# Manta-Network/manta-rs

Hardware: AMD Instinct MI355X
Metric: G1 MSM Mscalar/s at 2^20 (higher is better)
Workload: dtype u32; 1 GPU; 2^20 BLS12-381 G1 variable-base MSM per GPU, uniform scalars resident in HBM; curve=BLS12-381, log_n=20, window_bits=17, msms_in_flight=3

## Files before the change

include/mantagpu.h:

```cpp
#ifndef MANTAGPU_H
#define MANTAGPU_H
#include <stddef.h>
#include <stdint.h>

#ifdef __cplusplus
extern "C" {
#endif

typedef enum { MG_BN254 = 0, MG_BLS12_381 = 1 } mg_curve_t;

enum {
    MG_SUCCESS = 0,
    MG_ERROR_INVALID_ARGUMENT = 1,
    MG_ERROR_HIP = 2,
    MG_ERROR_OUT_OF_MEMORY = 3,
    MG_ERROR_DOMAIN_TOO_LARGE = 4,
    MG_ERROR_STATE = 5,
    MG_ERROR_CHECKSUM = 6
};

typedef struct mg_bases mg_bases;
typedef struct mg_msm_job mg_msm_job;
typedef struct mg_ctx mg_ctx;

// ... 22 lines not shown
int mg_bases_create_sharded(mg_curve_t curve, int group, const uint64_t *affine_mont, size_t n, const int *devices,
                            int n_devices, int precompute_window_bits, mg_bases **out);
int mg_bases_num_shards(const mg_bases *bases);
int mg_bases_shard(const mg_bases *bases, int shard, int *device, size_t *lo, size_t *hi);
void mg_bases_destroy(mg_bases *bases);
size_t mg_bases_device_bytes(const mg_bases *bases);
int mg_msm(const mg_bases *bases, const uint64_t *scalars_canonical, size_t n, uint64_t *out_affine_mont);
#define MG_SCALARS_MONT 1
#define MG_SCALARS_SPARSE 2
int mg_msm_launch(const mg_bases *bases, const uint64_t *d_scalars, size_t n, int scalar_flags, int window_bits,
                  mg_msm_job **job);
int mg_msm_launch_sharded(const mg_bases *bases, const uint64_t *const *d_scalars_per_shard, int scalar_flags,
                          int window_bits, mg_msm_job **job);
int mg_msm_finish(mg_msm_job *job, uint64_t *out_affine_mont);
int mg_msm_result_to_device(mg_msm_job *job, uint64_t *d_out_xyzz, void *stream);
size_t mg_xyzz_limbs(mg_curve_t curve, int group);
int mg_xyzz_sum(mg_curve_t curve, int group, const uint64_t *xyzz, size_t n, uint64_t *out_affine_mont);
int mg_points_sum(mg_curve_t curve, int group, const uint64_t *affine_mont, size_t n, uint64_t *out_affine_mont);
int mg_fixed_base_mul(mg_curve_t curve, int group, const uint64_t *base_affine_mont, const uint64_t *d_scalars,
                      size_t n, uint64_t *d_out_affine_mont);
#define MG_EC_ADD_MIXED 0
#define MG_EC_ADD 1
#define MG_EC_DOUBLE 2
#define MG_EC_MUL 3
#define MG_EC_SUB_MIXED 4
#define MG_EC_MUL_FIXED 5
int mg_ec_elementwise(mg_curve_t curve, int group, int op, const uint64_t *a_affine, const uint64_t *b, size_t n,
                      uint64_t *out_affine);
#define MG_FIELD_ADD 0
#define MG_FIELD_SUB 1
// ... 187 lines not shown
```

manta_rs_amd/api.py:

```python
from __future__ import annotations

import ctypes
import os

import numpy as np

_HERE = os.path.dirname(os.path.abspath(__file__))
LIB_PATH = os.environ.get("MANTA_LIB") or os.path.join(_HERE, "lib", "libmantagpu.so")

BN254, BLS12_381 = 0, 1
FQ_LIMBS = {BN254: 4, BLS12_381: 6}


class MantaGpuError(RuntimeError):

    def __init__(self, status, where=""):
        self.status = status
        detail = LIB.mg_last_error().decode() if status == 2 else ""
        super().__init__(f"{where}: {LIB.mg_strerror(status).decode()} ({status}) {detail}")


def _load():
    if not os.path.exists(LIB_PATH):
        raise ImportError(
# ... 30 lines not shown
    "mg_ntt_device", "mg_groth16_setup", "mg_ctx_create", "mg_ctx_create_from_bytes", "mg_ctx_set_r1cs", "mg_groth16_prove", "mg_groth16_prove_batch", "mg_witness_map", "mg_ctx_domain_size", "mg_ctx_table_bytes",
    "mg_ctx_destroy", "mg_bases_create_sharded", "mg_bases_num_shards", "mg_bases_shard", "mg_msm_launch_sharded",
    "mg_ctx_create_sharded", "mg_ctx_create_from_bytes_sharded", "mg_ctx_num_variables", "mg_ctx_num_inputs",
    "mg_ctx_num_shards", "mg_field_op", "mg_vk_create", "mg_vk_create_from_bytes", "mg_vk_encoded_size", "mg_vk_encode",
    "mg_vk_alpha_beta", "mg_vk_num_inputs", "mg_vk_destroy", "mg_groth16_verify", "mg_groth16_verify_batch", "mg_pairing_check", "mg_proof_decode", "mg_group_ntt",
    "mg_msm_result_to_device", "mg_xyzz_limbs", "mg_xyzz_sum", "mg_ctx_create_shard", "mg_partials_slot_limbs",
    "mg_groth16_partials_launch", "mg_groth16_partials_finish", "mg_groth16_assemble", "mg_blake3", "mg_ctx_create_from_bytes_checked",
    "mg_last_ntt_ms", "mg_hw_queues", "mg_last_prove_phases_ms", "mg_clock_probe", "mg_last_accumulate_mhz", "mg_ctx_create_task",
    "mg_ctx_opts_init", "mg_ctx_create_ex", "mg_ctx_create_from_bytes_ex", "mg_last_pass_host_ms",
    "mg_tuning_init", "mg_get_tuning", "mg_set_tuning", "mg_tuning_env_names",
    "mg_points_decode", "mg_points_check", "mg_points_encode", "mg_proofs_decode",
    "mg_poseidon_create", "mg_poseidon_destroy", "mg_poseidon_permute", "mg_poseidon_hash", "mg_poseidon_hash_device",
    "mg_merkle_tree", "mg_merkle_forest_roots",
    "mg_edwards_decode", "mg_edwards_encode", "mg_edwards_check", "mg_edwards_mul", "mg_edwards_add",
    "mg_note_cipher_create", "mg_note_cipher_destroy", "mg_notes_encrypt", "mg_notes_decrypt",
]


def _chk(rc, where):
    if rc != 0:
        raise MantaGpuError(rc, where)


def _p(a):
    return None if a is None else a.ctypes.data_as(_vp)


def _u64(a):
    return np.ascontiguousarray(a, dtype=np.uint64)

# ... 185 lines not shown


class MsmJob:
    def __init__(self, bases, handle):
        self.bases, self.handle = bases, handle

    def finish(self):
        out = np.zeros(affine_limbs(self.bases.curve, self.bases.group), dtype=np.uint64)
        _chk(LIB.mg_msm_finish(self.handle, _p(out)), "mg_msm_finish")
        self.handle = None
        return out

    def result_to_device(self, d_out_ptr, stream=None):
        _chk(LIB.mg_msm_result_to_device(self.handle, _addr(d_out_ptr), _addr(stream)), "mg_msm_result_to_device")

    def release(self):
        _chk(LIB.mg_msm_finish(self.handle, None), "mg_msm_finish")
        self.handle = None


class VariableBaseMSM:

    @staticmethod
    def multi_scalar_mul(bases: Bases, scalars) -> np.ndarray:
        sc = _u64(scalars)
        out = np.zeros(affine_limbs(bases.curve, bases.group), dtype=np.uint64)
        _chk(LIB.mg_msm(bases.handle, _p(sc), _sz(sc.shape[0]), _p(out)), "mg_msm")
        return out

    @staticmethod
# ... 1 lines not shown
        ptr = d_scalars.ptr if isinstance(d_scalars, DeviceBuffer) else d_scalars
        h = _vp()
        _chk(LIB.mg_msm_launch(bases.handle, ptr, _sz(n), int(bool(scalars_mont)) | (2 if sparse else 0), int(window_bits),
                               ctypes.byref(h)),
             "mg_msm_launch")
        return MsmJob(bases, h)

    @staticmethod
    def launch_sharded(bases: Bases, d_scalars_per_shard, scalars_mont=False, window_bits=0, sparse=False) -> MsmJob:
        ptrs = [d.ptr if isinstance(d, DeviceBuffer) else d for d in d_scalars_per_shard]
        arr = (_vp * len(ptrs))(*ptrs)
        h = _vp()
        _chk(LIB.mg_msm_launch_sharded(bases.handle, arr, int(bool(scalars_mont)) | (2 if sparse else 0), int(window_bits),
                                       ctypes.byref(h)), "mg_msm_launch_sharded")
        return MsmJob(bases, h)


def blake3(data: bytes) -> bytes:
    out = ctypes.create_string_buffer(32)
    _chk(LIB.mg_blake3(bytes(data), _sz(len(data)), out), "mg_blake3")
    return out.raw


def xyzz_limbs(curve, group) -> int:
    return int(LIB.mg_xyzz_limbs(curve, group))


def xyzz_sum(curve, group, xyzz) -> np.ndarray:
    pts = _u64(xyzz).reshape(-1, xyzz_limbs(curve, group))
    out = np.zeros(affine_limbs(curve, group), dtype=np.uint64)
# ... 707 lines not shown
```

manta_rs_amd/csrc/capi.cpp:

```cpp
#include "../../include/mantagpu.h"
#include "engine.h"
#include "staging.h"
#include "tuning.h"
#include <cstddef>
#include "prover.h"
#include "verify.h"
#include <cstring>
#include <new>
#include <vector>

using namespace mg;

struct BasesShard {
    GroupEngine *eng;
    BaseSet *bs;
    int device;
    size_t lo, hi;
};
struct mg_bases {
    std::vector<BasesShard> sh;
    size_t n = 0;
};
struct JobShard {
    GroupEngine *eng;
// ... 285 lines not shown
}
MG_API int mg_msm_result_to_device(mg_msm_job *job, uint64_t *d_out_xyzz, void *stream) {
    MG_TRY
    if (!job || job->sh.size() != 1 || !d_out_xyzz) return MG_ERROR_INVALID_ARGUMENT;
    JobShard &j = job->sh[0];
    DeviceGuard guard;
    MG_HIP(hipSetDevice(j.device));
    int rc = j.eng->msm_fold_device(j.ws, (u32 *)d_out_xyzz, (size_t)j.eng->xyzz_words());
    if (rc) return rc;
    hipStream_t ms = msm_stream_of(j.ws);
    MG_HIP(hipEventRecord(j.ws->done, ms));
    if ((hipStream_t)stream != ms) MG_HIP(hipStreamWaitEvent((hipStream_t)stream, j.ws->done, 0));
    return MG_SUCCESS;
    MG_CATCH
}
MG_API size_t mg_xyzz_limbs(mg_curve_t curve, int group) {
    GroupEngine *e = get_engine((int)curve, group);
    return e ? (size_t)e->xyzz_words() / 2 : 0;
}
MG_API int mg_xyzz_sum(mg_curve_t curve, int group, const uint64_t *xyzz, size_t n, uint64_t *out_affine) {
    MG_TRY
    GroupEngine *e = get_engine((int)curve, group);
    if (!e || !xyzz || !out_affine) return MG_ERROR_INVALID_ARGUMENT;
    HostPoint acc, t;
    e->hp_set_inf(&acc);
    for (size_t i = 0; i < n; ++i) {
        e->hp_from_xyzz(&t, (const u32 *)xyzz + i * (size_t)e->xyzz_words());
        e->hp_add(&acc, &t);
    }
    e->hp_to_affine(&acc, (u32 *)out_affine);
// ... 587 lines not shown
```

manta_rs_amd/csrc/engine.h:

```cpp
#pragma once
#include <hip/hip_runtime.h>
#include <shared_mutex>
#include <atomic>
#include <cstddef>
#include <cstdint>
#include <mutex>
#include <vector>

namespace mg {

typedef uint32_t u32;
typedef uint64_t u64;

#ifdef MG_NO_PRIO
#define MG_PRIO_HIGH() ((void)0)
#else
#define MG_PRIO_HIGH() __builtin_amdgcn_s_setprio(3)
#endif
#define MG_PRIO_FOR(F) MG_PRIO_HIGH()

enum { MG_OK = 0, MG_ERR_ARG = 1, MG_ERR_HIP = 2, MG_ERR_OOM = 3, MG_ERR_DOMAIN = 4, MG_ERR_STATE = 5 };

void set_last_hip_error(hipError_t e, const char *expr, const char *file, int line);
inline int hip_status(hipError_t e, const char *what, const char *file = __builtin_FILE(), int line = __builtin_LINE()) {
// ... 145 lines not shown
    bool use_solo = false;
    hipStream_t side_stream = nullptr;
    hipEvent_t side_fork = nullptr, side_join = nullptr;
    hipEvent_t done = nullptr;
    hipEvent_t t0 = nullptr, t1 = nullptr;
    bool timed = false;
    bool in_graph_slot = false;
    bool capturing = false;
    bool notify = false;
    u32 *h_flag = nullptr;
    u32 *d_token = nullptr;
    float accumulate_ms = 0.f;
    MsmPlan plan;
    MsmTail tail;
    u32 batch = 1;
    int pending = 0;
    int device = 0;
    ~MsmWorkspace();
};

inline hipStream_t msm_stream_of(const MsmWorkspace *ws) {
    return ws->run_on ? ws->run_on : (ws->use_solo && ws->solo ? ws->solo : ws->stream);
}

struct HostPoint {
    u64 w[4 * 12];
};

class GroupEngine {
  public:
// ... 48 lines not shown
    void ws_release(MsmWorkspace *);

    static constexpr size_t MAX_IDLE_WS = 24;

  protected:
    std::mutex ws_mu_;
    std::vector<MsmWorkspace *> ws_free_;
};

GroupEngine *make_engine_bn254_g1();
GroupEngine *make_engine_bn254_g2();
GroupEngine *make_engine_bls381_g1();
GroupEngine *make_engine_bls381_g2();
GroupEngine *get_engine(int curve, int group);

size_t sort_pairs_temp_bytes(size_t n);
bool sort_pairs_takes_device_count(int end_bit);
int sort_pairs(const u32 *keys_in, u32 *keys_out, const u32 *vals_in, u32 *vals_out, size_t n, int end_bit,
               void *tmp, size_t tmp_bytes, hipStream_t s, const u32 *d_count = nullptr, u32 lowmask = 0xffffffffu,
               u32 inv_from = 0xffffffffu);

}
```

manta_rs_amd/csrc/msm_digits.h:

```cpp
#pragma once
#include "msm_common.h"

namespace mg {

template <class FrC>
__global__ __launch_bounds__(1024) void digits_kernel(const u32 *__restrict__ scalars, u32 n, int c, int W, u32 B,
                                                     int precomp, u32 tstride, int mont, u32 invalid,
                                                     u32 *__restrict__ keys, u32 *__restrict__ vals,
                                                     const u32 *__restrict__ map, u32 n_scalars,
                                                     size_t scalar_stride, u32 seg_keys, u32 *__restrict__ count,
                                                     u32 n_sets = 1, u32 set_len = 0, u32 i_first = 0) {
    MG_PRIO_HIGH();
    const u32 i = i_first + blockIdx.x * blockDim.x + threadIdx.x;
    scalars += (size_t)blockIdx.y * scalar_stride;
    u32 src = (i < n) ? (map ? map[i] : i) : 0xffffffffu;
    u32 set = 0;
    if (n_sets > 1 && i < n) {
        set = src / set_len;
        src -= set * set_len;
    }
    const u32 key0 = (blockIdx.y * n_sets + set) * seg_keys;
    const bool have = i < n && src < n_scalars;
    u32 s[8] = {0, 0, 0, 0, 0, 0, 0, 0};
    if (have && mont == 2) {
        typedef FpR<FrC> R;
        const Fp<FrC> f = R::load(scalars + (size_t)src * R::K).to_canonical();
#pragma unroll
// ... 63 lines not shown
            const size_t o = (size_t)w * n + i;
            keys[o] = d ? key0 + (precomp == 2 ? 0u : precomp ? (d - 1) : ((u32)w * B + d - 1)) : invalid;
            vals[o] = d ? ((precomp == 2 ? ((u32)w * tstride + i) * B + (d - 1) : precomp ? ((u32)w * tstride + i) : i) | ((neg ^ flip) << 31)) : 0;
        }
        return;
    }
    const int lane = threadIdx.x & 63;
    u32 total = 0;
    {
        u32 t[8], carry = 0, neg;
#pragma unroll
        for (int j = 0; j < 8; ++j) t[j] = s[j];
        for (int w = 0; w < W; ++w) total += (u32)__popcll(__ballot(next_digit(t, carry, neg) != 0));
    }
    __shared__ u32 wave_tot[16], block_base;
    const int wv = threadIdx.x >> 6, nwv = blockDim.x >> 6;
    if (lane == 0) wave_tot[wv] = total;
    __syncthreads();
    if (threadIdx.x == 0) {
        u32 t = 0;
        for (int q = 0; q < nwv; ++q) t += wave_tot[q];
        block_base = t ? atomicAdd(count, t) : 0;
    }
    __syncthreads();
    u32 base = block_base;
    for (int q = 0; q < wv; ++q) base += wave_tot[q];
    const unsigned long long lt = (1ull << lane) - 1ull;
    u32 carry = 0, neg;
    for (int w = 0; w < W; ++w) {
        const u32 d = next_digit(s, carry, neg);
        const unsigned long long m = __ballot(d != 0);
        if (d) {
            const u32 o = base + (u32)__popcll(m & lt);
            keys[o] = key0 + (precomp == 2 ? 0u : precomp ? (d - 1) : ((u32)w * B + d - 1));
            vals[o] = (precomp == 2 ? ((u32)w * tstride + i) * B + (d - 1) : precomp ? ((u32)w * tstride + i) : i) | ((neg ^ flip) << 31);
        }
        base += (u32)__popcll(m);
    }
}

}
```

manta_rs_amd/csrc/msm_engine.h:

```cpp
#pragma once
#include "msm_common.h"
#include "staging.h"
#include "msm_digits.h"
#include "msm_accumulate.h"
#include "msm_reduce.h"
#include "msm_tables.h"

namespace mg {

template <class Curve, int GROUP> struct GT;
template <class Curve> struct GT<Curve, 1> {
#ifdef MG_G1_SATURATED
    typedef Fp<typename Curve::Fq> F;
#else
    typedef FpR<typename Curve::Fq> F;
#endif
    typedef Fp<typename Curve::Fq> FIO;
    typedef host::HFp<typename Curve::Fq> HF;
};
template <class Curve> struct GT<Curve, 2> {
#ifdef MG_G2_SATURATED
    typedef Fp2<typename Curve::Fq> F;
#else
    typedef Fp2R<typename Curve::Fq> F;
// ... 4 lines not shown

static inline u32 cdiv(size_t a, size_t b) { return (u32)((a + b - 1) / b); }

static __global__ __launch_bounds__(256) void stage_and_notify_kernel(const u32 *__restrict__ src0, u32 *__restrict__ dst0, u32 n0,
                                                                      const u32 *__restrict__ src1, u32 *__restrict__ dst1, u32 n1,
                                                                      u32 *__restrict__ flag) {
    for (u32 i = threadIdx.x; i < n0; i += 256) dst0[i] = src0[i];
    for (u32 i = threadIdx.x; i < n1; i += 256) dst1[i] = src1[i];
    __threadfence_system();
    __syncthreads();
    if (threadIdx.x == 0 && flag) {
        __atomic_store_n(flag, 1u, __ATOMIC_RELEASE);
        __threadfence_system();
    }
}
struct ZeroRanges {
    u32 *p[3];
    u32 n[3];
};
template <class F> __global__ __launch_bounds__(256) void zero_ranges(ZeroRanges r) {
    const u32 stride = gridDim.x * 256u, i0 = blockIdx.x * 256u + threadIdx.x;
#pragma unroll
    for (int t = 0; t < 3; ++t)
        for (u32 i = i0; i < r.n[t]; i += stride) r.p[t][i] = 0u;
}

static int ab_knob_in(const char *name, int lo, int hi, int dflt) {
    const int v = ab_knob(name, dflt);
    return v < lo ? lo : (v > hi ? hi : v);
}
struct MsmKnobs {
    int msm_L = ab_knob("MANTA_MSM_L", 0);
    int acc_round_waves = ab_knob("MANTA_ACC_ROUND_WAVES", -1);
    int coop_tiles = ab_knob("MANTA_COOP_TILES", 64);
    u32 coop_waves = (u32)ab_knob("MANTA_COOP_WAVES", 512);
    u32 merge_g = [](int v) { return (u32)(v >= 1 && v <= 64 ? v : 0); }(ab_knob("MANTA_MERGE_G", 0));
    int lgS0 = ab_knob_in("MANTA_RED_S0", 1, 8, 2), lgS = ab_knob_in("MANTA_RED_S", -1, 8, -1), lgSP = ab_knob_in("MANTA_RED_SP", 1, 8, 3);
    u32 min_items = (u32)ab_knob_in("MANTA_RED_MIN", 128, 1 << 30, 16384);
    u32 min_items_batch = (u32)ab_knob_in("MANTA_RED_MIN_BATCH", 128, 1 << 30, ab_knob("MANTA_RED_MIN", -1) >= 0 ? (int)min_items : 2048);
    bool side = ab_knob_in("MANTA_RED_SIDE", 0, 1, 1) != 0;
    bool sort_low = ab_knob("MANTA_SORT_LOW", 1) != 0;
    int acc_single = ab_knob("MANTA_ACC_SINGLE", 1);
    u32 digits_threads = [](int v) { return (u32)(v == 256 || v == 512 || v == 1024 ? v : 256); }(ab_knob("MANTA_DIGITS_THREADS", 0));
    bool z3_sort = ab_knob("MANTA_Z3_SORT", 0) != 0;
    size_t fixed_base_table_min = (size_t)ab_knob("MANTA_FIXED_BASE_TABLE_MIN", 16384);
};
static const MsmKnobs &msm_knobs() {
    static const MsmKnobs k;
    return k;
}

template <class Curve, int CURVE_ID, int GROUP> class GroupEngineT : public GroupEngine {
  public:
    typedef typename GT<Curve, GROUP>::F F;
    typedef typename GT<Curve, GROUP>::FIO FIO;
    typedef typename GT<Curve, GROUP>::HF HF;
    typedef host::HPoint<HF> HP;
    typedef typename Curve::Fr FrC;
    static constexpr int AW = Affine<F>::WORDS, XW = XYZZ<F>::WORDS;
// ... 566 lines not shown
    struct Launch {
        const BaseSet *bs;
        const u32 *d_scalars;
        MsmWorkspace *ws;
        hipStream_t s, side;
        size_t n, n_scalars, scalar_stride_words;
        int scalar_mode;
        u32 batch, nsets;
        bool batched_pass, sparse;
        MsmPlan pl;
        size_t M;
        int end_bit;
        u32 KB, seg_keys, nb, invalid, T, sort_mask = 0xffffffffu, sort_inv = 0xffffffffu;
        bool direct, per_query, acc_single;
        u32 *d_count;
        const u32 *skeys, *svals;
        u32 parts;
        const u32 *rin;
        u32 rstride, roff, rn;
        MsmTail tail;
    };

    int launch_reserve(Launch &r) {
        MsmWorkspace *const ws = r.ws; const MsmPlan &pl = r.pl;
        const size_t M = r.M = r.n * (size_t)pl.W * r.batch;
        r.KB = pl.full ? 1u : pl.B;
        if (M >= (1ull << 31) || (size_t)r.batch * r.nsets * pl.Wb * r.KB >= (1ull << 24)) return MG_ERR_ARG;
        if (pl.full) r.sparse = true;
        const u32 seg_keys = r.seg_keys = (u32)pl.Wb * r.KB;
        const u32 nb = r.nb = r.batch * r.nsets * seg_keys;
        const u32 invalid = r.invalid = nb;
        int rc;
        if ((rc = ws->keys_in.reserve(M * 4)) || (rc = ws->keys_out.reserve(M * 4)) ||
            (rc = ws->vals_in.reserve(M * 4)) || (rc = ws->vals_out.reserve(M * 4)))
            return rc;
        if ((rc = ws->sort_tmp.reserve(sort_pairs_temp_bytes(M))) || (rc = ws->buckets.reserve((size_t)(nb + 1) * XW * 4))) return rc;
        const u32 T = r.T = cdiv(M, pl.L);
        if ((rc = ws->pkeys[0].reserve((size_t)2 * T * 4)) || (rc = ws->ppts[0].reserve((size_t)2 * T * XW * 4)))
            return rc;
        const u32 waves1 = cdiv((size_t)2 * T, 64);
        if ((rc = ws->pkeys[1].reserve((size_t)2 * waves1 * 4)) ||
            (rc = ws->ppts[1].reserve((size_t)2 * waves1 * XW * 4)))
            return rc;

        if ((size_t)pl.W * r.bs->n * (pl.full ? pl.B : 1u) >= (1ull << 31)) return MG_ERR_ARG;
        int end_bit = 1;
        while ((1u << end_bit) <= invalid) ++end_bit;
        int end_bit_real = 1;
        while (nb > 1 && (1u << end_bit_real) <= nb - 1) ++end_bit_real;
        if ((end_bit + 7) / 8 > (end_bit_real + 7) / 8) r.sparse = true;
        if (r.sparse) end_bit = end_bit_real;
        if (msm_knobs().sort_low && !r.sparse && r.batch > 1 && r.nsets == 1 && (seg_keys & (seg_keys - 1)) == 0) {
            int eb = 1;
            while ((1u << eb) <= seg_keys) ++eb;
            if ((eb + 7) / 8 < (end_bit + 7) / 8) r.sort_mask = seg_keys - 1, r.sort_inv = invalid, end_bit = eb;
        }
        r.end_bit = end_bit;
        if (r.sparse && sort_pairs_takes_device_count(end_bit)) {
            if ((rc = ws->count.reserve(256))) return rc;
            r.d_count = ws->count.as<u32>();
        }
#ifdef MG_NO_DIRECT
        r.direct = false;
#else
        r.direct = nb == 1;
#endif
        if (r.direct && ((rc = ws->redA.reserve((size_t)XWM * 4)) || (rc = ws->redS.reserve((size_t)XWM * 4)))) return rc;
        ws->timed = kernel_timing() && !ws->capturing;
        if (ws->timed && !ws->h_clk) MG_HIP(hipHostMalloc((void **)&ws->h_clk, 64, hipHostMallocDefault));
        return MG_OK;
    }
    static constexpr int XWM = XW > XW_IO ? XW : XW_IO;

    void launch_digits(Launch &r) {
        MsmWorkspace *const ws = r.ws; const MsmPlan &pl = r.pl; const BaseSet *const bs = r.bs; hipStream_t s = r.s;
        ZeroRanges zr{};
        zr.p[0] = r.d_count, zr.n[0] = r.d_count ? 1u : 0u;
        zr.p[1] = r.direct ? ws->redS.as<u32>() : ws->buckets.as<u32>();
        zr.n[1] = r.direct ? (u32)XWM : (u32)((size_t)(r.nb + 1) * XW);
        zr.p[2] = ws->timed ? (u32 *)ws->h_clk : nullptr, zr.n[2] = ws->timed ? 4u : 0u;
        const u32 most = zr.n[1] > 4u ? zr.n[1] : 4u;
        hipLaunchKernelGGL((zero_ranges<F>), dim3(most > 256u * 1024u ? 1024u : cdiv(most, 256)), dim3(256), 0, s, zr);
        const u32 dthreads = r.d_count ? msm_knobs().digits_threads : 256u;
        const u32 nsets = r.nsets;
        r.per_query = pl.full && nsets > 1 && nsets <= BaseSet::MAX_SETS && r.batch == 1 && r.d_count && !msm_knobs().z3_sort &&
                      bs->set_first[nsets] == (u32)bs->n;
        if (r.per_query) {
            for (u32 q = 0; q < nsets; ++q) {
                const u32 lo = bs->set_first[q], hi = bs->set_first[q + 1];
                if (hi <= lo) continue;
                hipLaunchKernelGGL((digits_kernel<FrC>), dim3(cdiv(hi - lo, dthreads), 1), dim3(dthreads), 0, s, r.d_scalars, hi, pl.c,
                                   pl.W, pl.B, 2, (u32)bs->n, r.scalar_mode, r.invalid, ws->keys_in.as<u32>(), ws->vals_in.as<u32>(),
                                   (const u32 *)bs->d_map, (u32)r.n_scalars, r.scalar_stride_words, r.seg_keys, r.d_count, nsets,
                                   (u32)bs->set_len, lo);
            }
        } else
            hipLaunchKernelGGL((digits_kernel<FrC>), dim3(cdiv(r.n, dthreads), r.batch), dim3(dthreads), 0, s, r.d_scalars, (u32)r.n,
                               pl.c, pl.W, pl.B, pl.full ? 2 : (pl.precomp ? 1 : 0), (u32)bs->n, r.scalar_mode, r.invalid,
                               ws->keys_in.as<u32>(), ws->vals_in.as<u32>(), (const u32 *)bs->d_map, (u32)r.n_scalars,
                               r.scalar_stride_words, r.seg_keys, r.d_count, nsets, (u32)bs->set_len);
        r.batch *= nsets;
    }

    int launch_sort(Launch &r) {
        MsmWorkspace *const ws = r.ws;
        const bool no_sort = (r.nb == 1 || r.per_query) && r.d_count;
        r.skeys = no_sort ? ws->keys_in.as<u32>() : ws->keys_out.as<u32>();
        r.svals = no_sort ? ws->vals_in.as<u32>() : ws->vals_out.as<u32>();
        return no_sort ? MG_OK
                       : sort_pairs(ws->keys_in.as<u32>(), ws->keys_out.as<u32>(), ws->vals_in.as<u32>(), ws->vals_out.as<u32>(), r.M,
                                    r.end_bit, ws->sort_tmp.p, sort_pairs_temp_bytes(r.M), r.s, r.d_count, r.sort_mask, r.sort_inv);
    }

    int launch_accumulate(Launch &r) {
        MsmWorkspace *const ws = r.ws; const MsmPlan &pl = r.pl; const BaseSet *const bs = r.bs; hipStream_t s = r.s;
        u32 Tl = r.T, adapt = 0;
        u32 Lk = pl.L;
        const bool acc_single_on = ((msm_knobs().acc_single >> (GROUP - 1)) & 1) != 0;
        const int dev_now = current_device();
        const bool acc_single = r.acc_single = r.nb == 1 && r.d_count && acc_single_on && !(kernel_timing() && !ws->capturing) &&
                                               dev_now >= 0 && dev_now < 64 && occ_[dev_now].cus.load(std::memory_order_acquire) &&
                                               occ_[dev_now].blocks_single;
        if (r.d_count) {
            const u32 tgt = acc_round_lanes(r.batched_pass, acc_single);
            if (tgt && Tl > tgt) Tl = tgt, adapt = 1;
            else if (tgt && !r.batched_pass && pl.L > 6) adapt = 1;
// ... 174 lines not shown
```

manta_rs_amd/csrc/sort.hip:

```cpp
#include "engine.h"
#include <cstdlib>

namespace mg {

static constexpr int SORT_TILE = 4096;
static constexpr int SORT_ITEMS = 16;

__device__ __forceinline__ u32 sort_key(u32 k, u32 lowmask, u32 inv_from) { return k >= inv_from ? lowmask + 1u : (k & lowmask); }

__global__ __launch_bounds__(256) void radix_hist(const u32 *__restrict__ keys, u32 M, int shift, u32 ntiles,
                                                  u32 *__restrict__ hist, const u32 *__restrict__ count, u32 lowmask, u32 inv_from) {
    MG_PRIO_HIGH();
    if (count) M = *count;
    if ((size_t)blockIdx.x * SORT_TILE >= M) {
        hist[(size_t)threadIdx.x * ntiles + blockIdx.x] = 0;
        return;
    }
    __shared__ u32 cnt[256];
    cnt[threadIdx.x] = 0;
    __syncthreads();
    const size_t base = (size_t)blockIdx.x * SORT_TILE;
#pragma unroll
    for (int j = 0; j < SORT_ITEMS; ++j) {
        const size_t e = base + (size_t)j * 256 + threadIdx.x;
// ... 15 lines not shown
    __syncthreads();
    for (int d = 1; d < 256; d <<= 1) {
        const u32 v = threadIdx.x >= (u32)d ? part[threadIdx.x - d] : 0;
        __syncthreads();
        part[threadIdx.x] += v;
        __syncthreads();
    }
    u32 run = threadIdx.x ? part[threadIdx.x - 1] : 0;
    for (u32 i = lo; i < hi; ++i) {
        const u32 c = row[i];
        row[i] = run;
        run += c;
    }
    if (threadIdx.x == 255) totals[blockIdx.x] = part[255];
}
__global__ __launch_bounds__(256) void radix_scan_totals(u32 *__restrict__ totals) {
    MG_PRIO_HIGH();
    __shared__ u32 part[256];
    const u32 mine = totals[threadIdx.x];
    part[threadIdx.x] = mine;
    __syncthreads();
    for (int d = 1; d < 256; d <<= 1) {
        const u32 v = threadIdx.x >= (u32)d ? part[threadIdx.x - d] : 0;
        __syncthreads();
        part[threadIdx.x] += v;
        __syncthreads();
    }
    totals[threadIdx.x] = part[threadIdx.x] - mine;
}

__global__ __launch_bounds__(256) void radix_scatter(const u32 *__restrict__ keys_in, const u32 *__restrict__ vals_in,
                                                     u32 *__restrict__ keys_out, u32 *__restrict__ vals_out, u32 M,
                                                     int shift, u32 ntiles, const u32 *__restrict__ hist,
                                                     const u32 *__restrict__ totals, const u32 *__restrict__ count, u32 lowmask,
                                                     u32 inv_from) {
    MG_PRIO_HIGH();
    if (count) M = *count;
    if ((size_t)blockIdx.x * SORT_TILE >= M) return;
    __shared__ u32 wcount[4][256];
    __shared__ u32 gbase[256];
    __shared__ u32 sk[SORT_TILE], sv[SORT_TILE];
    const int wave = threadIdx.x >> 6, lane = threadIdx.x & 63;
#pragma unroll
    for (int w = 0; w < 4; ++w) wcount[w][threadIdx.x] = 0;
    __syncthreads();
    const size_t tile0 = (size_t)blockIdx.x * SORT_TILE;
    const size_t base = tile0 + (size_t)wave * (SORT_ITEMS * 64);
    u32 k[SORT_ITEMS], v[SORT_ITEMS];
    unsigned short rk[SORT_ITEMS];
    const unsigned long long lt_mask = (1ull << lane) - 1ull;
#pragma unroll
    for (int j = 0; j < SORT_ITEMS; ++j) {
        const size_t e = base + (size_t)j * 64 + lane;
        const bool valid = e < M;
        k[j] = valid ? keys_in[e] : 0u;
        v[j] = valid ? vals_in[e] : 0u;
        const u32 d = (sort_key(k[j], lowmask, inv_from) >> shift) & 255u;
        unsigned long long peers = __ballot(valid);
#pragma unroll
        for (int b = 0; b < 8; ++b) {
            const bool bit = (d >> b) & 1u;
            const unsigned long long bb = __ballot(bit);
            peers &= bit ? bb : ~bb;
        }
        const u32 before = wcount[wave][d];
        const u32 r = (u32)__popcll(peers & lt_mask);
        rk[j] = (unsigned short)(before + r);
        if (valid && r == 0) wcount[wave][d] = before + (u32)__popcll(peers);
    }
    __syncthreads();
    {
        const u32 d = threadIdx.x;
        const u32 c0 = wcount[0][d], c1 = wcount[1][d], c2 = wcount[2][d], c3 = wcount[3][d];
        const u32 tot = c0 + c1 + c2 + c3;
        gbase[d] = tot;
        __syncthreads();
        for (int s = 1; s < 256; s <<= 1) {
            const u32 x = d >= (u32)s ? gbase[d - s] : 0;
            __syncthreads();
            gbase[d] += x;
            __syncthreads();
        }
        const u32 loc = gbase[d] - tot;
        __syncthreads();
        wcount[0][d] = loc;
        wcount[1][d] = loc + c0;
        wcount[2][d] = loc + c0 + c1;
        wcount[3][d] = loc + c0 + c1 + c2;
        gbase[d] = hist[(size_t)d * ntiles + blockIdx.x] + totals[d] - loc;
    }
    __syncthreads();
#pragma unroll
    for (int j = 0; j < SORT_ITEMS; ++j) {
        const size_t e = base + (size_t)j * 64 + lane;
        if (e < M) {
            const u32 lp = wcount[wave][(sort_key(k[j], lowmask, inv_from) >> shift) & 255u] + rk[j];
            sk[lp] = k[j];
            sv[lp] = v[j];
        }
    }
    __syncthreads();
    const u32 cnt = tile0 >= M ? 0u : (u32)((tile0 + SORT_TILE <= M) ? SORT_TILE : (M - tile0));
    for (u32 t = threadIdx.x; t < cnt; t += 256) {
        const u32 kk = sk[t];
        const u32 pos = gbase[(sort_key(kk, lowmask, inv_from) >> shift) & 255u] + t;
        keys_out[pos] = kk;
        vals_out[pos] = sv[t];
    }
}

size_t sort_pairs_temp_bytes(size_t n) {
    const size_t ntiles = (n + SORT_TILE - 1) / SORT_TILE;
    return 2 * n * 4  + 256 * ntiles * 4 + 256 * 4 + 256;
}

bool sort_pairs_takes_device_count(int end_bit) { return end_bit >= 1 && end_bit <= 32; }

int sort_pairs(const u32 *keys_in, u32 *keys_out, const u32 *vals_in, u32 *vals_out, size_t n, int end_bit,
               void *tmp, size_t tmp_bytes, hipStream_t s, const u32 *d_count, u32 lowmask, u32 inv_from) {
    if (n == 0) return MG_OK;
    if (end_bit < 1 || end_bit > 32 || n >= (1ull << 32) || tmp_bytes < sort_pairs_temp_bytes(n)) return MG_ERR_ARG;
    const u32 M = (u32)n;
    const u32 ntiles = (u32)((n + SORT_TILE - 1) / SORT_TILE);
    const int passes = (end_bit + 7) / 8;
    u32 *tk = (u32 *)tmp, *tv = tk + n, *hist = tv + n, *totals = hist + (size_t)256 * ntiles;
    const u32 *ik = keys_in, *iv = vals_in;
    for (int p = 0; p < passes; ++p) {
        const bool to_out = ((passes - 1 - p) % 2) == 0;
        u32 *ok = to_out ? keys_out : tk, *ov = to_out ? vals_out : tv;
        hipLaunchKernelGGL(radix_hist, dim3(ntiles), dim3(256), 0, s, ik, M, 8 * p, ntiles, hist, d_count, lowmask, inv_from);
        hipLaunchKernelGGL(radix_scan_rows, dim3(256), dim3(256), 0, s, hist, ntiles, totals);
        hipLaunchKernelGGL(radix_scan_totals, dim3(1), dim3(256), 0, s, totals);
        hipLaunchKernelGGL(radix_scatter, dim3(ntiles), dim3(256), 0, s, ik, iv, ok, ov, M, 8 * p, ntiles, hist, totals, d_count, lowmask, inv_from);
        ik = ok;
        iv = ov;
    }
    MG_HIP(hipGetLastError());
    return MG_OK;
}

}
```

rust/mantagpu-sys/src/lib.rs:

```rust
#![no_std]
#![allow(non_camel_case_types)]

use core::ffi::{c_char, c_float, c_int, c_uint, c_void};

pub type mg_curve_t = c_int;
pub const MG_BN254: mg_curve_t = 0;
pub const MG_BLS12_381: mg_curve_t = 1;

pub const MG_SUCCESS: c_int = 0;
pub const MG_ERROR_INVALID_ARGUMENT: c_int = 1;
pub const MG_ERROR_HIP: c_int = 2;
pub const MG_ERROR_OUT_OF_MEMORY: c_int = 3;
pub const MG_ERROR_DOMAIN_TOO_LARGE: c_int = 4;
pub const MG_ERROR_STATE: c_int = 5;
pub const MG_ERROR_CHECKSUM: c_int = 6;
pub const MG_TASK_A: c_uint = 1;
pub const MG_TASK_B_G1: c_uint = 2;
pub const MG_TASK_B_G2: c_uint = 4;
pub const MG_TASK_L: c_uint = 8;
pub const MG_TASK_H: c_uint = 16;

pub const MG_SCALARS_MONT: c_int = 1;
pub const MG_SCALARS_SPARSE: c_int = 2;

// ... 185 lines not shown
        d_scalars: *const u64,
        n: usize,
        scalar_flags: c_int,
        window_bits: c_int,
        job: *mut *mut mg_msm_job,
    ) -> c_int;
    pub fn mg_msm_launch_sharded(
        bases: *const mg_bases,
        d_scalars_per_shard: *const *const u64,
        scalar_flags: c_int,
        window_bits: c_int,
        job: *mut *mut mg_msm_job,
    ) -> c_int;
    pub fn mg_msm_finish(job: *mut mg_msm_job, out_affine_mont: *mut u64) -> c_int;
    pub fn mg_msm_result_to_device(job: *mut mg_msm_job, d_out_xyzz: *mut u64, stream: *mut c_void) -> c_int;
    pub fn mg_xyzz_limbs(curve: mg_curve_t, group: c_int) -> usize;
    pub fn mg_xyzz_sum(curve: mg_curve_t, group: c_int, xyzz: *const u64, n: usize, out_affine_mont: *mut u64) -> c_int;
    pub fn mg_points_sum(curve: mg_curve_t, group: c_int, affine_mont: *const u64, n: usize, out_affine_mont: *mut u64) -> c_int;
    pub fn mg_fixed_base_mul(
        curve: mg_curve_t,
        group: c_int,
        base_affine_mont: *const u64,
        d_scalars: *const u64,
        n: usize,
        d_out_affine_mont: *mut u64,
    ) -> c_int;
    pub fn mg_ec_elementwise(
        curve: mg_curve_t,
        group: c_int,
        op: c_int,
// ... 247 lines not shown
```

Measured before the change: 409.1 Mscalar/s.

## Fuse first radix-sort histogram pass into digits kernel with per-block slices

The digits kernel now writes each block's pairs to a fixed slice, replacing the global atomic offset, and builds that block's 256-bin low-byte histogram in shared memory. The first sort pass then skips its radix_hist kernel and scatters straight from these per-block slices. The zero_ranges launch is folded into the digits kernel, and the totals scan is folded into the scatter kernel, which removes several kernel launches and one full read of the keys. The cost is shared-memory atomics in the digits kernel, a larger histogram buffer, and sparse slices in the unsorted output. New debug APIs expose the pair streams for testing.

```diff
diff --git a/include/mantagpu.h b/include/mantagpu.h
--- a/include/mantagpu.h
+++ b/include/mantagpu.h
@@ -60,6 +60,10 @@
                           int window_bits, mg_msm_job **job);
 int mg_msm_finish(mg_msm_job *job, uint64_t *out_affine_mont);
 int mg_msm_result_to_device(mg_msm_job *job, uint64_t *d_out_xyzz, void *stream);
+int mg_msm_job_pairs(mg_msm_job *job, int sorted, uint32_t *keys, uint32_t *vals, size_t capacity, size_t *n_pairs,
+                     uint32_t sort_key2[2]);
+int mg_sort_pairs(const uint32_t *keys, const uint32_t *vals, size_t n, int end_bit, uint32_t low_mask, uint32_t invalid_from,
+                  uint32_t *keys_out, uint32_t *vals_out);
 size_t mg_xyzz_limbs(mg_curve_t curve, int group);
 int mg_xyzz_sum(mg_curve_t curve, int group, const uint64_t *xyzz, size_t n, uint64_t *out_affine_mont);
 int mg_points_sum(mg_curve_t curve, int group, const uint64_t *affine_mont, size_t n, uint64_t *out_affine_mont);
diff --git a/manta_rs_amd/api.py b/manta_rs_amd/api.py
--- a/manta_rs_amd/api.py
+++ b/manta_rs_amd/api.py
@@ -68,6 +68,7 @@
     "mg_merkle_tree", "mg_merkle_forest_roots",
     "mg_edwards_decode", "mg_edwards_encode", "mg_edwards_check", "mg_edwards_mul", "mg_edwards_add",
     "mg_note_cipher_create", "mg_note_cipher_destroy", "mg_notes_encrypt", "mg_notes_decrypt",
+    "mg_msm_job_pairs", "mg_sort_pairs",
 ]
 
 
@@ -283,6 +284,13 @@
     def result_to_device(self, d_out_ptr, stream=None):
         _chk(LIB.mg_msm_result_to_device(self.handle, _addr(d_out_ptr), _addr(stream)), "mg_msm_result_to_device")
 
+    def pairs(self, sorted_stream):
+        n, sk = _sz(0), (ctypes.c_uint32 * 2)()
+        _chk(LIB.mg_msm_job_pairs(self.handle, int(sorted_stream), None, None, _sz(0), ctypes.byref(n), sk), "mg_msm_job_pairs")
+        k, v = np.zeros(max(n.value, 1), dtype=np.uint32), np.zeros(max(n.value, 1), dtype=np.uint32)
+        _chk(LIB.mg_msm_job_pairs(self.handle, int(sorted_stream), _p(k), _p(v), _sz(k.size), ctypes.byref(n), sk), "mg_msm_job_pairs")
+        return k[:n.value], v[:n.value], (int(sk[0]), int(sk[1]))
+
     def release(self):
         _chk(LIB.mg_msm_finish(self.handle, None), "mg_msm_finish")
         self.handle = None
@@ -314,6 +322,14 @@
         _chk(LIB.mg_msm_launch_sharded(bases.handle, arr, int(bool(scalars_mont)) | (2 if sparse else 0), int(window_bits),
                                        ctypes.byref(h)), "mg_msm_launch_sharded")
         return MsmJob(bases, h)
+
+
+def sort_pairs(keys, vals, end_bit, low_mask=0xFFFFFFFF, invalid_from=0xFFFFFFFF):
+    k, v = np.ascontiguousarray(keys, dtype=np.uint32), np.ascontiguousarray(vals, dtype=np.uint32)
+    ko, vo = np.zeros_like(k), np.zeros_like(v)
+    _chk(LIB.mg_sort_pairs(_p(k), _p(v), _sz(k.size), int(end_bit), ctypes.c_uint32(low_mask), ctypes.c_uint32(invalid_from), _p(ko), _p(vo)),
+         "mg_sort_pairs")
+    return ko, vo
 
 
 def blake3(data: bytes) -> bytes:
diff --git a/manta_rs_amd/csrc/capi.cpp b/manta_rs_amd/csrc/capi.cpp
--- a/manta_rs_amd/csrc/capi.cpp
+++ b/manta_rs_amd/csrc/capi.cpp
@@ -323,6 +323,66 @@
     return MG_SUCCESS;
     MG_CATCH
 }
+MG_API int mg_msm_job_pairs(mg_msm_job *job, int sorted, uint32_t *keys, uint32_t *vals, size_t capacity, size_t *n_pairs,
+                            uint32_t sort_key2[2]) {
+    MG_TRY
+    if (!job || job->sh.size() != 1 || !n_pairs) return MG_ERROR_INVALID_ARGUMENT;
+    JobShard &j = job->sh[0];
+    DeviceGuard guard;
+    MG_HIP(hipSetDevice(j.device));
+    MG_HIP(hipStreamSynchronize(msm_stream_of(j.ws)));
+    const MsmWorkspace::PairStream &ps = j.ws->pairs;
+    if (!ps.keys) return MG_ERROR_STATE;
+    if (sort_key2) sort_key2[0] = ps.sort_mask, sort_key2[1] = ps.sort_inv;
+    u32 n = ps.M;
+    if (ps.count) MG_HIP(memcpy_sync(&n, ps.count, 4, hipMemcpyDeviceToHost));
+    *n_pairs = n;
+    if (!keys || !vals) return MG_SUCCESS;
+    if (capacity < n) return MG_ERROR_INVALID_ARGUMENT;
+    if (sorted || !ps.rows) {
+        MG_HIP(memcpy_sync(keys, sorted ? ps.skeys : ps.keys, (size_t)n * 4, hipMemcpyDeviceToHost));
+        MG_HIP(memcpy_sync(vals, sorted ? ps.svals : ps.vals, (size_t)n * 4, hipMemcpyDeviceToHost));
+        return MG_SUCCESS;
+    }
+    std::vector<u32> sl((size_t)2 * ps.rows), k(ps.M), v(ps.M);
+    MG_HIP(memcpy_sync(sl.data(), ps.slices, sl.size() * 4, hipMemcpyDeviceToHost));
+    MG_HIP(memcpy_sync(k.data(), ps.keys, (size_t)ps.M * 4, hipMemcpyDeviceToHost));
+    MG_HIP(memcpy_sync(v.data(), ps.vals, (size_t)ps.M * 4, hipMemcpyDeviceToHost));
+    size_t o = 0;
+    for (u32 g = 0; g < ps.rows; ++g) {
+        const size_t at = sl[2 * g], cnt = sl[2 * g + 1];
+        if (at + cnt > ps.M || o + cnt > n) return MG_ERROR_STATE;
+        std::memcpy(keys + o, k.data() + at, cnt * 4);
+        std::memcpy(vals + o, v.data() + at, cnt * 4);
+        o += cnt;
+    }
+    return o == n ? MG_SUCCESS : MG_ERROR_STATE;
+    MG_CATCH
+}
+MG_API int mg_sort_pairs(const uint32_t *keys, const uint32_t *vals, size_t n, int end_bit, uint32_t low_mask, uint32_t invalid_from,
+                         uint32_t *keys_out, uint32_t *vals_out) {
+    MG_TRY
+    if (!keys || !vals || !keys_out || !vals_out || n == 0) return MG_ERROR_INVALID_ARGUMENT;
+    hipStream_t st = stream_pool_get_normal();
+    if (!st) return hip_status(hipErrorOutOfMemory, "mg_sort_pairs");
+    DevBlock m;
+    int rc = m.alloc({n * 4, n * 4, n * 4, n * 4, sort_pairs_temp_bytes(n)}, "mg_sort_pairs");
+    hipError_t e = hipSuccess;
+    if (!rc) {
+        e = hipMemcpyAsync(m.dev(0), keys, n * 4, hipMemcpyHostToDevice, st);
+        if (e == hipSuccess) e = hipMemcpyAsync(m.dev(1), vals, n * 4, hipMemcpyHostToDevice, st);
+        if (e == hipSuccess)
+            rc = sort_pairs(m.dev<u32>(0), m.dev<u32>(2), m.dev<u32>(1), m.dev<u32>(3), n, end_bit, m.dev(4), sort_pairs_temp_bytes(n), st,
+                            nullptr, low_mask, invalid_from);
+        if (e == hipSuccess && !rc) e = hipMemcpyAsync(keys_out, m.dev(2), n * 4, hipMemcpyDeviceToHost, st);
+        if (e == hipSuccess && !rc) e = hipMemcpyAsync(vals_out, m.dev(3), n * 4, hipMemcpyDeviceToHost, st);
+        const hipError_t e2 = hipStreamSynchronize(st);
+        if (e == hipSuccess) e = e2;
+    }
+    stream_pool_put_normal(st);
+    return rc ? rc : e == hipSuccess ? MG_SUCCESS : hip_status(e, "mg_sort_pairs");
+    MG_CATCH
+}
 MG_API size_t mg_xyzz_limbs(mg_curve_t curve, int group) {
     GroupEngine *e = get_engine((int)curve, group);
     return e ? (size_t)e->xyzz_words() / 2 : 0;
diff --git a/manta_rs_amd/csrc/engine.h b/manta_rs_amd/csrc/engine.h
--- a/manta_rs_amd/csrc/engine.h
+++ b/manta_rs_amd/csrc/engine.h
@@ -183,6 +183,11 @@
     MsmPlan plan;
     MsmTail tail;
     u32 batch = 1;
+    struct PairStream {
+        const u32 *keys = nullptr, *vals = nullptr, *skeys = nullptr, *svals = nullptr;
+        const u32 *count = nullptr, *slices = nullptr;
+        u32 rows = 0, M = 0, sort_mask = 0xffffffffu, sort_inv = 0xffffffffu;
+    } pairs;
     int pending = 0;
     int device = 0;
     ~MsmWorkspace();
@@ -261,10 +266,16 @@
 GroupEngine *make_engine_bls381_g2();
 GroupEngine *get_engine(int curve, int group);
 
-size_t sort_pairs_temp_bytes(size_t n);
+struct SortFirstPass {
+    u32 *hist, *slices;
+};
+size_t sort_pairs_temp_bytes(size_t n, size_t rows = 0);
+u32 sort_pairs_row_capacity();
+SortFirstPass sort_pairs_first_pass(void *tmp, size_t n, size_t rows);
 bool sort_pairs_takes_device_count(int end_bit);
 int sort_pairs(const u32 *keys_in, u32 *keys_out, const u32 *vals_in, u32 *vals_out, size_t n, int end_bit,
                void *tmp, size_t tmp_bytes, hipStream_t s, const u32 *d_count = nullptr, u32 lowmask = 0xffffffffu,
-               u32 inv_from = 0xffffffffu);
-
-}
+               u32 inv_from = 0xffffffffu,
+               u32 rows = 0, u32 *count_out = nullptr);
+
+}
diff --git a/manta_rs_amd/csrc/msm_digits.h b/manta_rs_amd/csrc/msm_digits.h
--- a/manta_rs_amd/csrc/msm_digits.h
+++ b/manta_rs_amd/csrc/msm_digits.h
@@ -2,6 +2,11 @@
 #include "msm_common.h"
 
 namespace mg {
+
+struct ZeroRanges {
+    u32 *p[3];
+    u32 n[3];
+};
 
 template <class FrC>
 __global__ __launch_bounds__(1024) void digits_kernel(const u32 *__restrict__ scalars, u32 n, int c, int W, u32 B,
@@ -9,8 +14,14 @@
                                                      u32 *__restrict__ keys, u32 *__restrict__ vals,
                                                      const u32 *__restrict__ map, u32 n_scalars,
                                                      size_t scalar_stride, u32 seg_keys, u32 *__restrict__ count,
-                                                     u32 n_sets = 1, u32 set_len = 0, u32 i_first = 0) {
+                                                     u32 n_sets = 1, u32 set_len = 0, u32 i_first = 0,
+                                                     u32 *__restrict__ row_hist = nullptr, u32 *__restrict__ row_slices = nullptr,
+                                                     ZeroRanges zr = ZeroRanges{}) {
     MG_PRIO_HIGH();
+    const u32 row = blockIdx.y * gridDim.x + blockIdx.x, nrows = gridDim.x * gridDim.y;
+#pragma unroll
+    for (int t = 0; t < 3; ++t)
+        for (u32 z = row * blockDim.x + threadIdx.x; z < zr.n[t]; z += nrows * blockDim.x) zr.p[t][z] = 0u;
     const u32 i = i_first + blockIdx.x * blockDim.x + threadIdx.x;
     scalars += (size_t)blockIdx.y * scalar_stride;
     u32 src = (i < n) ? (map ? map[i] : i) : 0xffffffffu;
@@ -104,13 +115,20 @@
         for (int w = 0; w < W; ++w) total += (u32)__popcll(__ballot(next_digit(t, carry, neg) != 0));
     }
     __shared__ u32 wave_tot[16], block_base;
+    __shared__ u32 low_cnt[256];
     const int wv = threadIdx.x >> 6, nwv = blockDim.x >> 6;
     if (lane == 0) wave_tot[wv] = total;
+    if (row_hist)
+        for (u32 t = threadIdx.x; t < 256u; t += blockDim.x) low_cnt[t] = 0u;
     __syncthreads();
     if (threadIdx.x == 0) {
         u32 t = 0;
         for (int q = 0; q < nwv; ++q) t += wave_tot[q];
-        block_base = t ? atomicAdd(count, t) : 0;
+        if (row_hist) {
+            block_base = (blockIdx.y * n + blockIdx.x * blockDim.x) * (u32)W;
+            row_slices[2 * row] = block_base, row_slices[2 * row + 1] = t;
+        } else
+            block_base = t ? atomicAdd(count, t) : 0;
     }
     __syncthreads();
     u32 base = block_base;
@@ -122,11 +140,17 @@
         const unsigned long long m = __ballot(d != 0);
         if (d) {
             const u32 o = base + (u32)__popcll(m & lt);
-            keys[o] = key0 + (precomp == 2 ? 0u : precomp ? (d - 1) : ((u32)w * B + d - 1));
+            const u32 key = key0 + (precomp == 2 ? 0u : precomp ? (d - 1) : ((u32)w * B + d - 1));
+            keys[o] = key;
+            if (row_hist) atomicAdd(&low_cnt[key & 255u], 1u);
             vals[o] = (precomp == 2 ? ((u32)w * tstride + i) * B + (d - 1) : precomp ? ((u32)w * tstride + i) : i) | ((neg ^ flip) << 31);
         }
         base += (u32)__popcll(m);
     }
+    if (row_hist) {
+        __syncthreads();
+        for (u32 t = threadIdx.x; t < 256u; t += blockDim.x) row_hist[(size_t)t * nrows + row] = low_cnt[t];
+    }
 }
 
 }
diff --git a/manta_rs_amd/csrc/msm_engine.h b/manta_rs_amd/csrc/msm_engine.h
--- a/manta_rs_amd/csrc/msm_engine.h
+++ b/manta_rs_amd/csrc/msm_engine.h
@@ -42,10 +42,6 @@
         __threadfence_system();
     }
 }
-struct ZeroRanges {
-    u32 *p[3];
-    u32 n[3];
-};
 template <class F> __global__ __launch_bounds__(256) void zero_ranges(ZeroRanges r) {
     const u32 stride = gridDim.x * 256u, i0 = blockIdx.x * 256u + threadIdx.x;
 #pragma unroll
@@ -71,6 +67,7 @@
     int acc_single = ab_knob("MANTA_ACC_SINGLE", 1);
     u32 digits_threads = [](int v) { return (u32)(v == 256 || v == 512 || v == 1024 ? v : 256); }(ab_knob("MANTA_DIGITS_THREADS", 0));
     bool z3_sort = ab_knob("MANTA_Z3_SORT", 0) != 0;
+    bool digits_rows = ab_knob("MANTA_DIGITS_ROWS", 1) != 0;
     size_t fixed_base_table_min = (size_t)ab_knob("MANTA_FIXED_BASE_TABLE_MIN", 16384);
 };
 static const MsmKnobs &msm_knobs() {
@@ -667,6 +664,7 @@
         u32 KB, seg_keys, nb, invalid, T, sort_mask = 0xffffffffu, sort_inv = 0xffffffffu;
         bool direct, per_query, acc_single;
         u32 *d_count;
+        u32 rows = 0;
         const u32 *skeys, *svals;
         u32 parts;
         const u32 *rin;
@@ -687,7 +685,7 @@
         if ((rc = ws->keys_in.reserve(M * 4)) || (rc = ws->keys_out.reserve(M * 4)) ||
             (rc = ws->vals_in.reserve(M * 4)) || (rc = ws->vals_out.reserve(M * 4)))
             return rc;
-        if ((rc = ws->sort_tmp.reserve(sort_pairs_temp_bytes(M))) || (rc = ws->buckets.reserve((size_t)(nb + 1) * XW * 4))) return rc;
+        if ((rc = ws->buckets.reserve((size_t)(nb + 1) * XW * 4))) return rc;
         const u32 T = r.T = cdiv(M, pl.L);
         if ((rc = ws->pkeys[0].reserve((size_t)2 * T * 4)) || (rc = ws->ppts[0].reserve((size_t)2 * T * XW * 4)))
             return rc;
@@ -712,7 +710,13 @@
         if (r.sparse && sort_pairs_takes_device_count(end_bit)) {
             if ((rc = ws->count.reserve(256))) return rc;
             r.d_count = ws->count.as<u32>();
-        }
+            const u32 dthreads = msm_knobs().digits_threads;
+            const bool per_query_set = pl.full && r.nsets > 1 && r.batch == 1;
+            if (msm_knobs().digits_rows && nb > 1 && !per_query_set && r.sort_mask == 0xffffffffu &&
+                (size_t)dthreads * pl.W <= sort_pairs_row_capacity())
+                r.rows = cdiv(r.n, dthreads) * r.batch;
+        }
+        if ((rc = ws->sort_tmp.reserve(sort_pairs_temp_bytes(M, r.rows)))) return rc;
 #ifdef MG_NO_DIRECT
         r.direct = false;
 #else
@@ -728,12 +732,13 @@
     void launch_digits(Launch &r) {
         MsmWorkspace *const ws = r.ws; const MsmPlan &pl = r.pl; const BaseSet *const bs = r.bs; hipStream_t s = r.s;
         ZeroRanges zr{};
-        zr.p[0] = r.d_count, zr.n[0] = r.d_count ? 1u : 0u;
+        zr.p[0] = r.rows ? nullptr : r.d_count, zr.n[0] = r.d_count && !r.rows ? 1u : 0u;
         zr.p[1] = r.direct ? ws->redS.as<u32>() : ws->buckets.as<u32>();
         zr.n[1] = r.direct ? (u32)XWM : (u32)((size_t)(r.nb + 1) * XW);
         zr.p[2] = ws->timed ? (u32 *)ws->h_clk : nullptr, zr.n[2] = ws->timed ? 4u : 0u;
         const u32 most = zr.n[1] > 4u ? zr.n[1] : 4u;
-        hipLaunchKernelGGL((zero_ranges<F>), dim3(most > 256u * 1024u ? 1024u : cdiv(most, 256)), dim3(256), 0, s, zr);
+        if (!r.rows) hipLaunchKernelGGL((zero_ranges<F>), dim3(most > 256u * 1024u ? 1024u : cdiv(most, 256)), dim3(256), 0, s, zr);
+        const SortFirstPass fp = r.rows ? sort_pairs_first_pass(ws->sort_tmp.p, r.M, r.rows) : SortFirstPass{nullptr, nullptr};
         const u32 dthreads = r.d_count ? msm_knobs().digits_threads : 256u;
         const u32 nsets = r.nsets;
         r.per_query = pl.full && nsets > 1 && nsets <= BaseSet::MAX_SETS && r.batch == 1 && r.d_count && !msm_knobs().z3_sort &&
@@ -751,7 +756,8 @@
             hipLaunchKernelGGL((digits_kernel<FrC>), dim3(cdiv(r.n, dthreads), r.batch), dim3(dthreads), 0, s, r.d_scalars, (u32)r.n,
                                pl.c, pl.W, pl.B, pl.full ? 2 : (pl.precomp ? 1 : 0), (u32)bs->n, r.scalar_mode, r.invalid,
                                ws->keys_in.as<u32>(), ws->vals_in.as<u32>(), (const u32 *)bs->d_map, (u32)r.n_scalars,
-                               r.scalar_stride_words, r.seg_keys, r.d_count, nsets, (u32)bs->set_len);
+                               r.scalar_stride_words, r.seg_keys, r.d_count, nsets, (u32)bs->set_len, 0u, fp.hist, fp.slices,
+                               r.rows ? zr : ZeroRanges{});
         r.batch *= nsets;
     }
 
@@ -760,9 +766,12 @@
         const bool no_sort = (r.nb == 1 || r.per_query) && r.d_count;
         r.skeys = no_sort ? ws->keys_in.as<u32>() : ws->keys_out.as<u32>();
         r.svals = no_sort ? ws->vals_in.as<u32>() : ws->vals_out.as<u32>();
+        ws->pairs = {ws->keys_in.as<u32>(), ws->vals_in.as<u32>(), r.skeys, r.svals, r.d_count,
+                     r.rows ? sort_pairs_first_pass(ws->sort_tmp.p, r.M, r.rows).slices : nullptr, r.rows, (u32)r.M, r.sort_mask, r.sort_inv};
         return no_sort ? MG_OK
                        : sort_pairs(ws->keys_in.as<u32>(), ws->keys_out.as<u32>(), ws->vals_in.as<u32>(), ws->vals_out.as<u32>(), r.M,
-                                    r.end_bit, ws->sort_tmp.p, sort_pairs_temp_bytes(r.M), r.s, r.d_count, r.sort_mask, r.sort_inv);
+                                    r.end_bit, ws->sort_tmp.p, sort_pairs_temp_bytes(r.M, r.rows), r.s, r.rows ? nullptr : r.d_count,
+                                    r.sort_mask, r.sort_inv, r.rows, r.rows ? r.d_count : nullptr);
     }
 
     int launch_accumulate(Launch &r) {
diff --git a/manta_rs_amd/csrc/sort.hip b/manta_rs_amd/csrc/sort.hip
--- a/manta_rs_amd/csrc/sort.hip
+++ b/manta_rs_amd/csrc/sort.hip
@@ -53,37 +53,27 @@
     }
     if (threadIdx.x == 255) totals[blockIdx.x] = part[255];
 }
-__global__ __launch_bounds__(256) void radix_scan_totals(u32 *__restrict__ totals) {
-    MG_PRIO_HIGH();
-    __shared__ u32 part[256];
-    const u32 mine = totals[threadIdx.x];
-    part[threadIdx.x] = mine;
-    __syncthreads();
-    for (int d = 1; d < 256; d <<= 1) {
-        const u32 v = threadIdx.x >= (u32)d ? part[threadIdx.x - d] : 0;
-        __syncthreads();
-        part[threadIdx.x] += v;
-        __syncthreads();
-    }
-    totals[threadIdx.x] = part[threadIdx.x] - mine;
-}
 
 __global__ __launch_bounds__(256) void radix_scatter(const u32 *__restrict__ keys_in, const u32 *__restrict__ vals_in,
                                                      u32 *__restrict__ keys_out, u32 *__restrict__ vals_out, u32 M,
                                                      int shift, u32 ntiles, const u32 *__restrict__ hist,
                                                      const u32 *__restrict__ totals, const u32 *__restrict__ count, u32 lowmask,
-                                                     u32 inv_from) {
+                                                     u32 inv_from, const u32 *__restrict__ slices, u32 *__restrict__ count_out) {
     MG_PRIO_HIGH();
     if (count) M = *count;
-    if ((size_t)blockIdx.x * SORT_TILE >= M) return;
+    size_t tile0 = (size_t)blockIdx.x * SORT_TILE;
+    u32 cnt = tile0 >= M ? 0u : (u32)((tile0 + SORT_TILE <= M) ? SORT_TILE : (M - tile0));
+    if (slices) tile0 = slices[2 * blockIdx.x], cnt = slices[2 * blockIdx.x + 1];
+    const size_t tend = tile0 + cnt;
+    if (cnt == 0 && !(count_out && blockIdx.x == 0)) return;
     __shared__ u32 wcount[4][256];
     __shared__ u32 gbase[256];
+    __shared__ u32 tsum[256];
     __shared__ u32 sk[SORT_TILE], sv[SORT_TILE];
     const int wave = threadIdx.x >> 6, lane = threadIdx.x & 63;
 #pragma unroll
     for (int w = 0; w < 4; ++w) wcount[w][threadIdx.x] = 0;
     __syncthreads();
-    const size_t tile0 = (size_t)blockIdx.x * SORT_TILE;
     const size_t base = tile0 + (size_t)wave * (SORT_ITEMS * 64);
     u32 k[SORT_ITEMS], v[SORT_ITEMS];
     unsigned short rk[SORT_ITEMS];
@@ -91,7 +81,7 @@
 #pragma unroll
     for (int j = 0; j < SORT_ITEMS; ++j) {
         const size_t e = base + (size_t)j * 64 + lane;
-        const bool valid = e < M;
+        const bool valid = e < tend;
         k[j] = valid ? keys_in[e] : 0u;
         v[j] = valid ? vals_in[e] : 0u;
         const u32 d = (sort_key(k[j], lowmask, inv_from) >> shift) & 255u;
@@ -111,35 +101,38 @@
     {
         const u32 d = threadIdx.x;
         const u32 c0 = wcount[0][d], c1 = wcount[1][d], c2 = wcount[2][d], c3 = wcount[3][d];
-        const u32 tot = c0 + c1 + c2 + c3;
+        const u32 tot = c0 + c1 + c2 + c3, rtot = totals[d];
         gbase[d] = tot;
+        tsum[d] = rtot;
         __syncthreads();
         for (int s = 1; s < 256; s <<= 1) {
-            const u32 x = d >= (u32)s ? gbase[d - s] : 0;
+            const u32 x = d >= (u32)s ? gbase[d - s] : 0, y = d >= (u32)s ? tsum[d - s] : 0;
             __syncthreads();
             gbase[d] += x;
+            tsum[d] += y;
             __syncthreads();
         }
         const u32 loc = gbase[d] - tot;
+        const u32 first = tsum[d] - rtot;
+        if (count_out && blockIdx.x == 0 && d == 255) *count_out = tsum[255];
         __syncthreads();
         wcount[0][d] = loc;
         wcount[1][d] = loc + c0;
         wcount[2][d] = loc + c0 + c1;
         wcount[3][d] = loc + c0 + c1 + c2;
-        gbase[d] = hist[(size_t)d * ntiles + blockIdx.x] + totals[d] - loc;
+        gbase[d] = hist[(size_t)d * ntiles + blockIdx.x] + first - loc;
     }
     __syncthreads();
 #pragma unroll
     for (int j = 0; j < SORT_ITEMS; ++j) {
         const size_t e = base + (size_t)j * 64 + lane;
-        if (e < M) {
+        if (e < tend) {
             const u32 lp = wcount[wave][(sort_key(k[j], lowmask, inv_from) >> shift) & 255u] + rk[j];
             sk[lp] = k[j];
             sv[lp] = v[j];
         }
     }
     __syncthreads();
-    const u32 cnt = tile0 >= M ? 0u : (u32)((tile0 + SORT_TILE <= M) ? SORT_TILE : (M - tile0));
     for (u32 t = threadIdx.x; t < cnt; t += 256) {
         const u32 kk = sk[t];
         const u32 pos = gbase[(sort_key(kk, lowmask, inv_from) >> shift) & 255u] + t;
@@ -148,29 +141,45 @@
     }
 }
 
-size_t sort_pairs_temp_bytes(size_t n) {
+static size_t sort_hist_cols(size_t n, size_t rows) {
     const size_t ntiles = (n + SORT_TILE - 1) / SORT_TILE;
-    return 2 * n * 4  + 256 * ntiles * 4 + 256 * 4 + 256;
+    return rows > ntiles ? rows : ntiles;
+}
+size_t sort_pairs_temp_bytes(size_t n, size_t rows) {
+    return 2 * n * 4  + 256 * sort_hist_cols(n, rows) * 4 + 256 * 4 + 2 * rows * 4 + 256;
+}
+u32 sort_pairs_row_capacity() { return SORT_TILE; }
+SortFirstPass sort_pairs_first_pass(void *tmp, size_t n, size_t rows) {
+    u32 *hist = (u32 *)tmp + 2 * n;
+    return SortFirstPass{hist, hist + 256 * sort_hist_cols(n, rows) + 256};
 }
 
 bool sort_pairs_takes_device_count(int end_bit) { return end_bit >= 1 && end_bit <= 32; }
 
 int sort_pairs(const u32 *keys_in, u32 *keys_out, const u32 *vals_in, u32 *vals_out, size_t n, int end_bit,
-               void *tmp, size_t tmp_bytes, hipStream_t s, const u32 *d_count, u32 lowmask, u32 inv_from) {
+               void *tmp, size_t tmp_bytes, hipStream_t s, const u32 *d_count, u32 lowmask, u32 inv_from, u32 rows, u32 *count_out) {
     if (n == 0) return MG_OK;
-    if (end_bit < 1 || end_bit > 32 || n >= (1ull << 32) || tmp_bytes < sort_pairs_temp_bytes(n)) return MG_ERR_ARG;
+    if (end_bit < 1 || end_bit > 32 || n >= (1ull << 32) || tmp_bytes < sort_pairs_temp_bytes(n, rows)) return MG_ERR_ARG;
+    if (rows && (!count_out || lowmask != 0xffffffffu)) return MG_ERR_ARG;
     const u32 M = (u32)n;
     const u32 ntiles = (u32)((n + SORT_TILE - 1) / SORT_TILE);
     const int passes = (end_bit + 7) / 8;
-    u32 *tk = (u32 *)tmp, *tv = tk + n, *hist = tv + n, *totals = hist + (size_t)256 * ntiles;
+    u32 *tk = (u32 *)tmp, *tv = tk + n, *hist = tv + n, *totals = hist + 256 * sort_hist_cols(n, rows), *slices = totals + 256;
     const u32 *ik = keys_in, *iv = vals_in;
     for (int p = 0; p < passes; ++p) {
         const bool to_out = ((passes - 1 - p) % 2) == 0;
         u32 *ok = to_out ? keys_out : tk, *ov = to_out ? vals_out : tv;
-        hipLaunchKernelGGL(radix_hist, dim3(ntiles), dim3(256), 0, s, ik, M, 8 * p, ntiles, hist, d_count, lowmask, inv_from);
-        hipLaunchKernelGGL(radix_scan_rows, dim3(256), dim3(256), 0, s, hist, ntiles, totals);
-        hipLaunchKernelGGL(radix_scan_totals, dim3(1), dim3(256), 0, s, totals);
-        hipLaunchKernelGGL(radix_scatter, dim3(ntiles), dim3(256), 0, s, ik, iv, ok, ov, M, 8 * p, ntiles, hist, totals, d_count, lowmask, inv_from);
+        if (p == 0 && rows) {
+            hipLaunchKernelGGL(radix_scan_rows, dim3(256), dim3(256), 0, s, hist, rows, totals);
+            hipLaunchKernelGGL(radix_scatter, dim3(rows), dim3(256), 0, s, ik, iv, ok, ov, M, 0, rows, hist, totals, (const u32 *)nullptr, lowmask,
+                               inv_from, slices, count_out);
+            d_count = count_out;
+        } else {
+            hipLaunchKernelGGL(radix_hist, dim3(ntiles), dim3(256), 0, s, ik, M, 8 * p, ntiles, hist, d_count, lowmask, inv_from);
+            hipLaunchKernelGGL(radix_scan_rows, dim3(256), dim3(256), 0, s, hist, ntiles, totals);
+            hipLaunchKernelGGL(radix_scatter, dim3(ntiles), dim3(256), 0, s, ik, iv, ok, ov, M, 8 * p, ntiles, hist, totals, d_count, lowmask,
+                               inv_from, (const u32 *)nullptr, (u32 *)nullptr);
+        }
         ik = ok;
         iv = ov;
     }
diff --git a/rust/mantagpu-sys/src/lib.rs b/rust/mantagpu-sys/src/lib.rs
--- a/rust/mantagpu-sys/src/lib.rs
+++ b/rust/mantagpu-sys/src/lib.rs
@@ -223,6 +223,25 @@
     ) -> c_int;
     pub fn mg_msm_finish(job: *mut mg_msm_job, out_affine_mont: *mut u64) -> c_int;
     pub fn mg_msm_result_to_device(job: *mut mg_msm_job, d_out_xyzz: *mut u64, stream: *mut c_void) -> c_int;
+    pub fn mg_msm_job_pairs(
+        job: *mut mg_msm_job,
+        sorted: c_int,
+        keys: *mut u32,
+        vals: *mut u32,
+        capacity: usize,
+        n_pairs: *mut usize,
+        sort_key2: *mut u32,
+    ) -> c_int;
+    pub fn mg_sort_pairs(
+        keys: *const u32,
+        vals: *const u32,
+        n: usize,
+        end_bit: c_int,
+        low_mask: u32,
+        invalid_from: u32,
+        keys_out: *mut u32,
+        vals_out: *mut u32,
+    ) -> c_int;
     pub fn mg_xyzz_limbs(curve: mg_curve_t, group: c_int) -> usize;
     pub fn mg_xyzz_sum(curve: mg_curve_t, group: c_int, xyzz: *const u64, n: usize, out_affine_mont: *mut u64) -> c_int;
     pub fn mg_points_sum(curve: mg_curve_t, group: c_int, affine_mont: *const u64, n: usize, out_affine_mont: *mut u64) -> c_int;
```

Measured after the change: 409.9 Mscalar/s, median of 3. No clear change (+0.2%).
